# HKUST-KnowComp/DualMessagePassing

Hardware: AMD Instinct MI355X
Metric: (pattern,graph) pairs/sec DMPNN fwd+bwd hid=128 (higher is better)
Workload: dtype f32

## Files before the change

### dualmessagepassing_amd/_abi.py

```python
import ctypes

c_int = ctypes.c_int
c_i32 = ctypes.c_int32
c_i64 = ctypes.c_int64
c_u64 = ctypes.c_uint64
c_f32 = ctypes.c_float
c_double = ctypes.c_double
c_ptr = ctypes.c_void_p
c_size = ctypes.c_size_t

ABI_VERSION = 91

DMP_COLLATE_MAX_JOBS = 4
DMP_POOL_MAX_JOBS = 4
DMP_REDUCE_MAX_SEGMENTS = 16
DMP_ADAMW_MAX_SKIP = 16
DMP_ADAMW_MAX_SEGMENTS = 1024
DMP_LOOKUP_MAX_JOBS = 8
DMP_CONCAT_MAX_JOBS = 12
DMP_GEMM_MAX_JOBS = 12
DMP_GEMM_MAX_TERMS = 3
DMP_ATB_MAX_JOBS = 8
DMP_MEM_MEAN, DMP_MEM_SUM, DMP_MEM_MAX = 0, 1, 2


class dmp_collate_job(ctypes.Structure):
# ... 80 lines not shown

class dmp_head_io(ctypes.Structure):
    _fields_ = [("ps", c_ptr), ("ld_ps", c_i64), ("gs", c_ptr), ("ld_gs", c_i64), ("pl", c_ptr), ("gl", c_ptr), ("scale_p", c_f32),
                ("scale_g", c_f32), ("F", c_ptr), ("Y1S", c_ptr), ("y", c_ptr)]


class dmp_head_grads(ctypes.Structure):
    _fields_ = [("dy", c_ptr), ("dy_scale", c_ptr), ("dY1", c_ptr), ("dP", c_ptr), ("dG", c_ptr), ("dps", c_ptr), ("ld_dps", c_i64),
                ("dgs", c_ptr), ("ld_dgs", c_i64), ("dWp", c_ptr), ("dbp", c_ptr), ("dWg", c_ptr), ("dbg", c_ptr), ("dW1", c_ptr),
                ("db1", c_ptr), ("dW2", c_ptr), ("db2", c_ptr)]


class dmp_typed_job(ctypes.Structure):
    _fields_ = [("Hin", c_ptr), ("ldh", c_i64), ("W2", c_ptr), ("ldw", c_i64), ("w_in_out", c_int), ("bias", c_ptr), ("R", c_ptr),
                ("ldr", c_i64), ("R2", c_ptr), ("ldr2", c_i64), ("act", c_int), ("slope", c_f32), ("out", c_ptr), ("ldo", c_i64)]


class dmp_atb2_job(ctypes.Structure):
    _fields_ = [("Z", c_ptr), ("ldz", c_i64), ("D", c_ptr), ("ldd", c_i64), ("partial_T", c_ptr), ("partial_B", c_ptr),
                ("partial_stride", c_i64), ("ldp", c_int)]


class dmp_atb_job(ctypes.Structure):
    _fields_ = [("A", c_ptr), ("lda", c_i64), ("B", c_ptr), ("ldb", c_i64), ("gate", c_ptr), ("partial", c_ptr), ("partial_stride", c_i64),
                ("ldp", c_int), ("partial_colsum", c_ptr), ("cs_ld", c_int), ("rowmask", c_ptr)]


_p = ctypes.POINTER


# ... 159 lines not shown
    "dmp_l0_bwd_w_rows": (c_int, [c_ptr, c_i64, c_int, c_ptr, c_ptr, c_i64, c_ptr, c_i64, c_ptr, c_ptr, c_i64, c_int, c_ptr, c_ptr]),
    "dmp_typed_partial_rows": (c_i64, [c_i64, c_int]),
    "dmp_out_fwd_typed": (c_int, [_p(dmp_typed_job), c_int, c_ptr, c_ptr, c_ptr, c_i64, c_i64, c_int, c_ptr]),
    "dmp_bwd_h1_typed": (c_int, [c_ptr, c_i64, c_ptr, c_i64, c_ptr, c_i64, c_ptr, c_ptr, c_ptr, c_i64, c_i64, c_int, c_f32, c_ptr, c_i64,
                                 c_ptr, c_ptr, c_ptr]),
    "dmp_kept_rows_jobs": (c_int, [_p(dmp_kept_job), c_int, c_ptr, c_ptr, c_ptr, c_ptr, c_i64, c_ptr, c_ptr, c_ptr, c_ptr]),
    "dmp_row_mask_bits_jobs": (c_int, [_p(dmp_rowmask_job), c_int, c_ptr]),
    "dmp_atb2_blocks": (c_i64, [c_i64, c_int]),
    "dmp_atb2_jobs": (c_int, [_p(dmp_atb2_job), c_int, c_ptr, c_ptr, c_ptr, c_i64, c_i64, c_int, c_ptr]),
    "dmp_bwd_z_w": (c_int, [c_ptr, c_i64, c_ptr, c_i64, c_ptr, c_i64, c_ptr, c_i64, c_i64, c_ptr, c_i64, c_ptr, c_ptr, c_f32, c_f32,
                            c_ptr, c_ptr, c_ptr, c_i64, c_i64, c_int, c_ptr, c_i64, c_ptr, c_i64, c_ptr, c_ptr]),
    "dmp_out_fwd_typed_codes": (c_int, [_p(dmp_typed_job), c_ptr, c_i64, c_int, c_ptr, c_i64, c_i64, c_i64, c_ptr, c_ptr, c_ptr, c_i64, c_i64, c_int, c_ptr]),
    "dmp_bwd_h1_w_blocks": (c_i64, [c_i64]),
    "dmp_bwd_h1_w": (c_int, [c_ptr, c_i64, c_ptr, c_i64, c_ptr, c_i64, c_ptr, c_ptr, c_i64, c_i64, c_int, c_f32, c_ptr, c_i64,
                             c_ptr, c_ptr, c_ptr, c_ptr]),
    "dmp_row_mask_bits": (c_int, [c_ptr, c_i64, c_ptr, c_ptr]),
    "dmp_row_mask_rows": (c_int, [c_ptr, c_i64, c_int, c_i64, c_ptr, c_ptr]),
    "dmp_bwd_z_fused": (c_int, [c_ptr, c_i64, c_ptr, c_i64, c_ptr, c_i64, c_i64, c_ptr, c_i64, c_ptr, c_ptr, c_ptr,
                                c_f32, c_f32, c_i64, c_int, c_ptr, c_i64, c_ptr]),
    "dmp_gemm_k128": (c_int, [c_ptr, c_i64, c_ptr, c_i64, c_int, c_ptr, c_i64, c_i64, c_int, c_ptr]),
    "dmp_edge_combine": (c_int, [c_ptr, c_i64, c_ptr, c_i64, c_ptr, c_ptr, c_ptr, c_ptr, c_ptr, c_i64,
                                 c_int, c_int, c_f32, c_ptr, c_i64, c_ptr]),
    "dmp_relu_bwd_g_colsum": (c_int, [c_ptr, c_i64, c_ptr, c_i64, c_ptr, c_ptr, c_i64, c_int, c_f32, c_ptr, c_i64,
                                      c_ptr, c_ptr]),
    "dmp_edge_combine_bwd_g": (c_int, [c_ptr, c_i64, c_ptr, c_ptr, c_i64, c_int, c_ptr, c_i64, c_ptr]),
    "dmp_compgcn_agg": (c_int, [c_ptr, c_i64, c_ptr, c_i64, c_ptr, c_ptr, c_ptr, c_ptr, c_i64, c_int, c_int,
                                c_ptr, c_i64, c_ptr]),
    "dmp_compgcn_agg_bwd": (c_int, [c_ptr, c_i64, c_ptr, c_i64, c_ptr, c_i64, c_ptr, c_ptr, c_ptr, c_ptr,
                                    c_i64, c_int, c_int, c_ptr, c_i64, c_ptr, c_i64, c_ptr]),
    "dmp_attn_supported_dh": (c_int, [c_int]),
# ... 24 lines not shown
```

### dualmessagepassing_amd/_build.py

```python
import fcntl
import hashlib
import os
import shutil
import subprocess
import tempfile

_HERE = os.path.dirname(os.path.abspath(__file__))
CSRC = os.path.join(_HERE, "csrc")
LIB_PATH = os.path.join(CSRC, "libdmp_hip.so")
HASH_PATH = LIB_PATH + ".srchash"
SOURCES = ["dmp_agg.hip", "dmp_segacc.hip", "dmp_compact.hip", "dmp_graph.hip", "dmp_fused.hip", "dmp_mfma.hip", "dmp_typed.hip", "dmp_h1w.hip", "dmp_atb.hip", "dmp_fold.hip", "dmp_heads.hip", "dmp_layer0.hip", "dmp_bn.hip", "dmp_attn.hip", "dmp_mem.hip", "dmp_cnn.hip", "dmp_rnn.hip", "dmp_relconv.hip", "dmp_relcorr.hip",
           "dmp_subiso.cpp"]
HEADERS = ["dmp_common.h", "dmp_mfma_common.h", os.path.join("..", "..", "include", "dmp_hip.h")]
ARCH = "gfx950"
FLAGS = ["-O3", "-std=c++17", "-fPIC", "-ffp-contract=off", "-Wall", "-Wno-unused-function"]


def find_hipcc():
    for cand in (os.environ.get("HIPCC"), shutil.which("hipcc"), "/opt/rocm/bin/hipcc"):
        if cand and os.path.exists(cand):
            return cand
    return None


def source_hash():
    h = hashlib.sha256()
# ... 61 lines not shown
```

### dualmessagepassing_amd/fused.py

```python
import threading

import torch
from torch.autograd.function import once_differentiable

from . import _abi, _lib, ops
from ._lib import check, ptr, stream_ptr


def _partials(rows, H, dev):
    lib = _lib.load()
    return torch.empty((int(lib.dmp_colsum_partial_rows(rows, H)), H), dtype=torch.float32, device=dev)


MAX_REDUCE_SEGMENTS = _abi.DMP_REDUCE_MAX_SEGMENTS


class _Deferred(threading.local):

    def __init__(self):
        self.stack = []


_deferred = _Deferred()

# ... 657 lines not shown

def bwd_h1_typed(d_o, W2, h1, tiles, slope=0.0, out=None):
    lib = _lib.load()
    E, H = d_o.shape
    slot_edge, tile_scale, num_tiles, bound = tiles
    d_g = out if out is not None else dead_rows_buffer((E, H), d_o.device)
    G = int(lib.dmp_typed_partial_rows(bound, H))
    part = torch.empty((G, H), dtype=torch.float32, device=d_o.device)
    part_rows = torch.empty_like(part)
    W2 = W2.contiguous()
    with _lib.timed("bwd_h1_typed[H=%d,E=%d]", (H, E), 12 * H * E + 4 * E):
        check(lib.dmp_bwd_h1_typed(ptr(d_o), d_o.stride(0), ptr(W2), W2.size(1), ptr(h1), h1.stride(0), ptr(slot_edge), ptr(tile_scale),
                                   ptr(num_tiles), bound, E, H, slope, ptr(d_g), d_g.stride(0), ptr(part), ptr(part_rows), stream_ptr()),
              "dmp_bwd_h1_typed")
    return d_g, reduce_partials(part), reduce_partials(part_rows)


def h1w_ok(d_o, h1, H):
    lib = _lib.load()
    return (H == 128 and not lib.dmp_dev_get_exact_fp32() and d_o.size(0) * d_o.stride(0) * 4 < (1 << 32) - 65536
            and h1.size(0) * h1.stride(0) * 4 < (1 << 32) - 65536 and d_o.size(0) * H * 4 < (1 << 32) - 65536)


def bwd_h1_w(d_o, W2, h1, tiles, slope=0.0, out=None):
    lib = _lib.load()
    E, H = d_o.shape
    slot_edge, _, num_tiles, bound = tiles
    d_g = out if out is not None else dead_rows_buffer((E, H), d_o.device)
    G = int(lib.dmp_bwd_h1_w_blocks(bound))
    part = torch.empty((G, H), dtype=torch.float32, device=d_o.device)
# ... 704 lines not shown
    @staticmethod
    def forward(ctx, index, coef, residual, x, z, v_gate, e_gate, Bn, bn, Wx, Wes, be, nW2, nb2, eW2, eb2,
                WesT=None, nW2t=None, eW2t=None, slope=0.0, vpool=None, epool=None, l0=None, W0=None, WV0=None, edge_rows=True,
                inner=0):
        _lib.require_gpu(x, z)
        H = Bn.size(1)
        x, z = x.contiguous(), z.contiguous()
        Bn, Wx, Wes = Bn.contiguous(), Wx.contiguous(), Wes.contiguous()
        N = index.num_nodes
        from . import side
        side.wait("nodes")
        nd = node_rows(index, v_gate, H) if (N >= 4096 and onepanel_ok(H)) else None
        if nd is not None and l0 is not None and any(n0 % 32 for _, _, (n0, _) in l0.tables(z.size(0), N)):
            nd = None
        S0 = M0 = tables = None
        if l0 is not None:
            enc0, K0 = l0.enc, l0.K
            tables = l0.tables(z.size(0), N)
            if nd is not None and enc0.size(1) % 4 == 0:
                S0 = ops.seg_sum_raw(enc0, index.in_ptr, index.in_ent, N, None, True, -1.0, 1.0,
                                     out=dead_rows_buffer((N, 2 * enc0.size(1)), z.device), rows=nd.rows, tag="seg_sum2_codes")
            else:
                S0 = ops.seg_sum_raw(enc0, index.in_ptr, index.in_ent, N, None, True, -1.0, 1.0)
            Kp = enc0.size(1)
            vcodes_f = l0.venc is not None
            node_pass = (vcodes_f and H in MFMA_WIDTHS and l0.VK + 2 * K0 <= L0_NODE_MAX_COLS and W0.size(0) // K0 <= 2)
            TK = W0.size(0)
            M0 = torch.empty((TK, 2 * H), dtype=torch.float32, device=z.device)
            jobs = [(M0, [(W0, False, Wes, False)], None)]
            if node_pass:
# ... 28 lines not shown
                        SB[n0:n1].addmm_(S0[n0:n1, Kp:Kp + K0], WB[1, t * K0:(t + 1) * K0])
            S = None
        else:
            side.wait("keepcsr")
            kc = keep_in_csr(index, e_gate) if zero_rows_gate(e_gate) else None
            if kc is not None and nd is not None:
                S = ops.seg_sum_raw(z, kc[0], kc[1], N, None, True, -1.0, 1.0, out=dead_rows_buffer((N, 2 * H), z.device), rows=nd.rows)
            elif kc is not None:
                S = ops.seg_sum_raw(z, kc[0], kc[1], N, None, True, -1.0, 1.0)
            else:
                S = ops.seg_sum_raw(z, index.in_ptr, index.in_ent, N, e_gate.reshape(-1) if zero_rows_gate(e_gate) else None, True, -1.0, 1.0)
            if nd is None:
                SB = S @ Bn
        if l0 is None and nd is not None:
            T = nd.tiles
            XP = dead_rows_buffer((N, 3 * H), z.device)
            T1 = dead_rows_buffer((N, H), z.device)
            H1n = dead_rows_buffer((N, H), z.device)
            typed_jobs([dict(a=x, W=Wx[:, :H], bias=bn, out=XP[:, :H]), dict(a=S[:, :H], W=Bn[:H], out=T1),
                        dict(a=x, W=Wx[:, H:2 * H], out=XP[:, H:2 * H]), dict(a=x, W=Wx[:, 2 * H:], out=XP[:, 2 * H:])], T)
            out_fwd_typed(S[:, H:], Bn[H:], None, XP[:, :H], T, out=H1n, slope=slope, prev2=T1)
        elif l0 is not None and node_pass:
            pass
        elif l0 is not None and l0.venc is not None:
            VK = l0.VK
            XP = torch.empty((N, 3 * H), dtype=torch.float32, device=z.device)
            for t, (n0, n1) in l0.vtables(N):
                smallk_embed(l0.venc[n0:n1, :VK], MV[t * VK:(t + 1) * VK], None, XP[n0:n1], H)
        else:
            XP = x @ Wx
        if l0 is not None and node_pass:
            PXr, ldpx = PX, 2 * H
        else:
            PXr, ldpx = XP[:, H:], 3 * H
            if l0 is not None or nd is None:
                H1n = add_bias_relu_(SB, XP[:, :H], bn, slope)
        if nd is not None:
            xn = dead_rows_buffer((N, H), z.device) if (inner & 1) else torch.zeros((N, H), dtype=torch.float32, device=z.device)
            if nW2t is not None:
                out_fwd_typed(H1n, nW2t, nb2, x if residual else None, nd.tiles, out=xn)
            else:
                out_fwd_typed(H1n, nW2, nb2, x if residual else None, nd.tiles, out=xn, w_in_out=False)
        elif onepanel_ok(H):
            xn = out_fwd_mfma(H1n, nW2, nb2, v_gate, x if residual else None, nW2t)
        else:
            xn = gate_residual(x if residual else None, torch.addmm(nb2, H1n, nW2.t()), v_gate)
        sums_only = epool is not None and not edge_rows
        zn = None
        side.wait("erows" if l0 is not None else "tiles")
        dead_gate = e_gate if (SKIP_DEAD_ROWS and USE_ROW_MASKS and e_gate is not None and typed_ok(index, H)
                               and gate_row_mask(e_gate) is not None) else None
        if l0 is not None:
# ... 22 lines not shown
                if l0 is not None and residual and getattr(l0, "z_from_codes", False) and out_codes_ok(H1e, l0.enc, l0.K, W0[-l0.K:]):
                    zn = out_fwd_typed_codes(H1e, eW2t, eb2, l0.enc, l0.K, W0[-l0.K:], tl_, prev=l0.z_head, row0=l0.z_head.size(0))
                else:
                    zn = out_fwd_typed(H1e, eW2t, eb2, l0_rows(l0, W0, z) if residual else None, tl_)
            elif (l0 is not None and residual and e_gate is None and getattr(l0, "z_from_codes", False) and eW2t is not None
                  and out_codes_ok(H1e, l0.enc, l0.K, W0[-l0.K:]) and identity_tiles(H1e.size(0), H1e.device) is not None):
                zn = out_fwd_typed_codes(H1e, eW2t, eb2, l0.enc, l0.K, W0[-l0.K:], identity_tiles(H1e.size(0), H1e.device), prev=l0.z_head,
                                         row0=l0.z_head.size(0))
            else:
                zn = out_fwd_mfma(H1e, eW2, eb2, e_gate, l0_rows(l0, W0, z) if residual else None, eW2t, dead_rows=dead)
        ctx.index, ctx.coef, ctx.residual, ctx.H = index, coef, residual, H
        ctx.v_gate, ctx.e_gate, ctx.WesT, ctx.slope = v_gate, e_gate, WesT, slope
        ctx.vpool, ctx.epool = vpool, epool
        ctx.inner = int(inner)
        ctx.nd = nd
        ctx.l0, ctx.l0_S0, ctx.l0_tables = l0, S0, tables
        ctx.l0_W = None if l0 is None else (W0.detach(), None if WV0 is None else WV0.detach())
        ctx.save_for_backward(x, z if l0 is None else None, S, H1n, H1e, Bn, Wx, Wes, nW2, eW2)
        if vpool is None and epool is None:
            return xn, zn
        ctx.set_materialize_grads(False)
        vs = pool_rows(xn, vpool) if vpool is not None else None
        if sums_only:
            halves = 2 if epool.flag8 is not None else 1
            G_ = epool.num_graphs
            Q = pool_rows(H1e, epool, e_gate).view(G_ * halves, H)
            cnt = pool_weight_sums(epool, e_gate)
            ctx.gcnt = cnt
            cnt = cnt.view(G_ * halves, 1)
            zs = pool_rows(z, epool, e_gate if zero_rows_gate(e_gate) else None).view(G_ * halves, H) if residual else None
# ... 102 lines not shown
                XX = (torch.empty if full else torch.zeros)((TK, (3 if ctx.residual else 2) * H), dtype=torch.float32, device=dG.device)
                for t, rows, _ in tables:
                    if rows[1] > rows[0]:
                        l0_bwd_w(l0.enc, K0, ix.edge_select(coef)[2], dG, dzn if ctx.residual else None, rows, XX[t * K0:(t + 1) * K0],
                                 mask=(gate_row_mask(ctx.e_gate) if (getattr(l0, "enc_mask", None) is not None and binary_gate_mask(ctx.e_gate) is not None)
                                       else getattr(l0, "enc_mask", None)))
                dWes = None
            else:
                fuse_dzw = bool(typed and ctx.needs_input_grad[4] and H == 128 and
                                (ctx.e_gate is None or (SKIP_DEAD_ROWS and zero_rows_gate(ctx.e_gate) and live_tiles(ix, coef, ctx.e_gate) is not None)))
                dWes = None if fuse_dzw else (atb_typed(z, dG, coef, ix, gate=ctx.e_gate) if typed else atb(z, dG))
            wg = (lambda a, b: atb_rows(a, b, colsum=False)[0]) if atb_ok(x, dXP) else atb
            one_launch = onepanel_ok(H) and atb_ok(dxn, H1n) and atb_ok(x, dXP) and (l0 is not None or atb_ok(S, dXP))
            if nd is not None and not (one_launch and binary_gate_mask(ctx.v_gate) is not None):
                raise _lib.DmpError("fused layer backward: the kept-node path needs the masked weight-gradient launch")
            if nd is not None:
                dPn, dbn, db2n = bwd_h1_typed(dxn, nW2, H1n, nd.tiles, slope, out=dXP[:, :H])
                if vcodes:
                    dW2n = atb_rows(dxn, H1n, ctx.v_gate, colsum=False)[0]
            elif onepanel_ok(H) and atb_ok(dxn, H1n):
                if binary_gate_mask(ctx.v_gate) is not None:
                    dPn, dbn, db2n = bwd_h1_mfma(dxn, nW2, H1n, both_halves=False, gate=ctx.v_gate, out=dXP[:, :H], slope=slope,
                                                 rows_colsum=True)
                    if not one_launch or vcodes:
                        dW2n = atb_rows(dxn, H1n, ctx.v_gate, colsum=False)[0]
                else:
                    if not one_launch or vcodes:
                        dW2n, db2n = atb_rows(dxn, H1n, ctx.v_gate)
                    dPn, dbn = bwd_h1_mfma(dxn, nW2, H1n, both_halves=False, gate=ctx.v_gate, out=dXP[:, :H], slope=slope)
            else:
                dOn, db2n = scale_rows_colsum(dxn, ctx.v_gate)
# ... 26 lines not shown
                        klist = nd.rows if (nd is not None and n0 == 0 and n1 == N) else None
                        smallk_atb_cols(l0.venc[n0:n1, :VK], dXP[n0:n1], dxn[n0:n1] if ctx.residual else None,
                                        Yn[:, t * VK:(t + 1) * VK], H,
                                        mask=vmask[n0 // 32:] if (klist is None and vmask is not None and n0 % 32 == 0) else None, rows=klist)
                elif one_launch:
                    vm = binary_gate_mask(ctx.v_gate)
                    if nd is not None:
                        (dW2n, _), (dWx, _) = atb_rows_multi([(dxn, H1n, None, False), (x, dXP, None, False)], tiles=nd.tiles)
                    elif vm is not None:
                        (dW2n, _), (dWx, _) = atb_rows_multi([(dxn, H1n, None, False, vm), (x, dXP, None, False)])
                    else:
                        (dW2n, db2n), (dWx, _) = atb_rows_multi([(dxn, H1n, ctx.v_gate, True, gate_row_mask(ctx.v_gate)), (x, dXP, None, False)])
                else:
                    dWx = wg(x, dXP)
            else:
                if nd is not None:
                    dS = dead_rows_buffer((N, 2 * H), x.device)
                    jobs = [dict(a=dPn, W=Bn[:H], w_in_out=False, out=dS[:, :H]), dict(a=dPn, W=Bn[H:], w_in_out=False, out=dS[:, H:])]
                    if ctx.needs_input_grad[3]:
                        dxU = dead_rows_buffer((N, 2 * H), x.device)
                        jobs += [dict(a=dXP[:, :H], W=Wx[:, :H], w_in_out=False, prev=dxn if ctx.residual else None, out=dxU[:, :H]),
                                 dict(a=dXP[:, H:2 * H], W=Wx[:, H:2 * H], w_in_out=False, out=dxU[:, H:])]
                    typed_jobs(jobs, nd.tiles)
                else:
                    dS = dPn @ Bn.t()
                if one_launch:
                    vm = gate_row_mask(ctx.v_gate)
                    if nd is not None:
                        (dW2n, _), (dBn, _), (dWx, _) = atb_rows_multi([(dxn, H1n, None, False), (S, dPn, None, False), (x, dXP, None, False)],
                                                                        tiles=nd.tiles)
                    elif binary_gate_mask(ctx.v_gate) is not None:
                        (dW2n, _), (dBn, _), (dWx, _) = atb_rows_multi([(dxn, H1n, None, False, vm), (S, dPn, None, False, vm),
                                                                         (x, dXP, None, False)])
                    else:
                        (dW2n, db2n), (dBn, _), (dWx, _) = atb_rows_multi([(dxn, H1n, ctx.v_gate, True, vm), (S, dPn, None, False, vm),
                                                                            (x, dXP, None, False)])
                else:
                    dBn = wg(S, dPn)
                    dWx = wg(x, dXP)
            dx = None
            if ctx.needs_input_grad[3] and nd is not None:
                dx = dead_rows_buffer((N, H), x.device) if (ctx.inner & 2) else torch.zeros((N, H), dtype=torch.float32, device=x.device)
                if l0 is None:
                    out_fwd_typed(dXP[:, 2 * H:], Wx[:, 2 * H:], None, dxU[:, :H], nd.tiles, out=dx, w_in_out=False, prev2=dxU[:, H:])
                else:
                    for b3 in range(3):
                        out_fwd_typed(dXP[:, b3 * H:(b3 + 1) * H], Wx[:, b3 * H:(b3 + 1) * H], None,
                                      (dxn if ctx.residual else None) if b3 == 0 else dx, nd.tiles, out=dx, w_in_out=False)
            elif ctx.needs_input_grad[3]:
                dx = torch.addmm(dxn, dXP, Wx.t()) if ctx.residual else dXP @ Wx.t()
            dz = None
            if l0 is None and ctx.needs_input_grad[4]:
                dead_dz = (("leave" if (ctx.inner & 2) else "zero") if (typed and SKIP_DEAD_ROWS and zero_rows_gate(ctx.e_gate)) else None)
                dst_m = None if nd is None else nd.sel[2]
                both = None
                if typed and dWes is None:
# ... 88 lines not shown
```

### include/dmp_hip.h

```cpp
#ifndef DMP_HIP_H
#define DMP_HIP_H

#include <stddef.h>
#include <stdint.h>

#ifdef __cplusplus
extern "C" {
#endif

#define DMP_OK 0
#define DMP_ERR_BAD_ARG (-1)
#define DMP_ERR_UNSUPPORTED (-2)
#define DMP_ERR_HIP (-3)

#define DMP_ABI_VERSION 91
int dmp_abi_version(void);
const char *dmp_last_hip_error(void);


size_t dmp_csr_workspace_words(int64_t num_nodes, int64_t num_edges);

int dmp_csr_build(const int64_t *key, const uint8_t *flag, int64_t num_edges,
                  int64_t num_nodes, int32_t *rowptr, int32_t *ent,
                  int32_t *key32, int64_t *degree, int32_t *status,
                  int32_t *ws, void *stream);

size_t dmp_csr_pair_workspace_words(int64_t num_nodes);
int dmp_csr_build_pair(const int64_t *dst, const int64_t *src, const uint8_t *flag, int64_t num_edges, int64_t num_nodes,
                       int32_t *in_ptr, int32_t *in_ent, int32_t *dst32, int64_t *in_deg,
                       int32_t *out_ptr, int32_t *out_ent, int32_t *src32, int64_t *out_deg,
// ... 469 lines not shown
  float *partial_T, *partial_B; int64_t partial_stride; int ldp;
} dmp_atb2_job;
int64_t dmp_atb2_blocks(int64_t tiles_bound, int num_jobs);
int dmp_atb2_jobs(const dmp_atb2_job *jobs, int num_jobs, const int32_t *slot_row, const float *tile_scale, const int32_t *num_tiles,
                  int64_t tiles_bound, int64_t rows, int H, void *stream);

int dmp_bwd_z_w(const float *dPre, int64_t ldp, const float *Z, int64_t ldz, const float *W, int64_t ldw, const float *D, int64_t ldd,
                int64_t num_nodes, const float *base, int64_t ldb, const int32_t *dst, const uint8_t *flag, float s0, float s1,
                const int32_t *slot_edge, const float *tile_scale, const int32_t *num_tiles, int64_t tiles_bound, int64_t E, int H,
                const int32_t *base_map, int64_t base_rows, float *dZ, int64_t ldo, float *partial_w, void *stream);
int64_t dmp_bwd_h1_w_blocks(int64_t tiles_bound);
int dmp_bwd_h1_w(const float *dO, int64_t ldo, const float *W2, int64_t ldw, const float *H1, int64_t ldh,
                 const int32_t *slot_edge, const int32_t *num_tiles, int64_t tiles_bound, int64_t E, int H, float slope,
                 float *dG, int64_t ldg, float *partial, float *partial_rows, float *partial_w, void *stream);

int dmp_bwd_z_fused(const float *dPre, int64_t ldp, const float *W, int64_t ldw,
                    const float *D, int64_t ldd, int64_t num_nodes, const float *base, int64_t ldb,
                    const float *coefE, const int32_t *dst, const uint8_t *flag, float s0,
                    float s1, int64_t num_edges, int H, float *dZ, int64_t ldz, void *stream);

int dmp_edge_fwd_typed(const float *Z, int64_t ldz, const float *W, int64_t ldw, const float *P,
                       int64_t ldp, int64_t num_nodes, const float *bias, const int32_t *selA,
                       const int32_t *selB, const int32_t *slot_edge, const float *tile_scale,
                       const int32_t *num_tiles, int64_t tiles_bound, int64_t num_edges, int H,
                       float slope, float *H1, int64_t ldh, void *stream);
int dmp_mask_slots(const int32_t *slot, int64_t n, const float *gate, int64_t E, int32_t *out, void *stream);
int dmp_bwd_z_typed_arow(const float *dPre, int64_t ldp, const float *W, int64_t ldw, const float *D, int64_t ldd,
                         int64_t num_nodes, const float *base, int64_t ldb, const int32_t *dst, const uint8_t *flag,
                         float s0, float s1, const int32_t *slot_edge, const int32_t *slot_arow, const float *tile_scale,
                         const int32_t *num_tiles, int64_t tiles_bound, int64_t E, int H, int w_transposed,
// ... 93 lines not shown
```

Measured before the change: 469,800.

## Fuse node-side typed GEMM chain into single persistent MFMA kernel for fwd and bwd

Adds a node_chain kernel that runs the whole per-node chain (x/S projections, bias+activation, second linear layer with residual) for each 128-row tile in one launch. It keeps intermediates in LDS as split-bf16 images and streams packed weight panels double-buffered. In backward it also fuses activation-gradient, dS/dx products and column sums. This replaces several typed_jobs/out_fwd_typed launches and their intermediate global round-trips, at the cost of a large LDS footprint, limited occupancy, and an extra weight-packing pass each call.

After: 486,500, median of 6. +3.5%, better.

```diff
diff --git a/dualmessagepassing_amd/_abi.py b/dualmessagepassing_amd/_abi.py
--- a/dualmessagepassing_amd/_abi.py
+++ b/dualmessagepassing_amd/_abi.py
@@ -9,7 +9,7 @@
 c_ptr = ctypes.c_void_p
 c_size = ctypes.c_size_t
 
-ABI_VERSION = 91
+ABI_VERSION = 92
 
 DMP_COLLATE_MAX_JOBS = 4
 DMP_POOL_MAX_JOBS = 4
@@ -120,6 +120,10 @@
 class dmp_typed_job(ctypes.Structure):
     _fields_ = [("Hin", c_ptr), ("ldh", c_i64), ("W2", c_ptr), ("ldw", c_i64), ("w_in_out", c_int), ("bias", c_ptr), ("R", c_ptr),
                 ("ldr", c_i64), ("R2", c_ptr), ("ldr2", c_i64), ("act", c_int), ("slope", c_f32), ("out", c_ptr), ("ldo", c_i64)]
+
+
+class dmp_chain_panel(ctypes.Structure):
+    _fields_ = [("W", c_ptr), ("ld", c_i64), ("transposed", c_int)]
 
 
 class dmp_atb2_job(ctypes.Structure):
@@ -309,6 +313,13 @@
     "dmp_bwd_h1_w_blocks": (c_i64, [c_i64]),
     "dmp_bwd_h1_w": (c_int, [c_ptr, c_i64, c_ptr, c_i64, c_ptr, c_i64, c_ptr, c_ptr, c_i64, c_i64, c_int, c_f32, c_ptr, c_i64,
                              c_ptr, c_ptr, c_ptr, c_ptr]),
+    "dmp_node_chain_blocks": (c_i64, [c_i64]),
+    "dmp_node_chain_panel_words": (c_i64, []),
+    "dmp_node_chain_pack": (c_int, [_p(dmp_chain_panel), c_int, c_ptr, c_ptr]),
+    "dmp_node_chain_fwd": (c_int, [c_ptr, c_i64, c_ptr, c_i64, c_ptr, c_ptr, c_ptr, c_int, c_f32, c_ptr, c_ptr, c_i64, c_i64, c_int,
+                                   c_ptr, c_i64, c_ptr, c_i64, c_ptr, c_i64, c_ptr]),
+    "dmp_node_chain_bwd": (c_int, [c_ptr, c_i64, c_ptr, c_i64, c_ptr, c_i64, c_ptr, c_int, c_f32, c_ptr, c_ptr, c_i64, c_i64, c_int,
+                                   c_ptr, c_i64, c_ptr, c_i64, c_ptr, c_i64, c_ptr, c_ptr, c_ptr]),
     "dmp_row_mask_bits": (c_int, [c_ptr, c_i64, c_ptr, c_ptr]),
     "dmp_row_mask_rows": (c_int, [c_ptr, c_i64, c_int, c_i64, c_ptr, c_ptr]),
     "dmp_bwd_z_fused": (c_int, [c_ptr, c_i64, c_ptr, c_i64, c_ptr, c_i64, c_i64, c_ptr, c_i64, c_ptr, c_ptr, c_ptr,
diff --git a/dualmessagepassing_amd/_build.py b/dualmessagepassing_amd/_build.py
--- a/dualmessagepassing_amd/_build.py
+++ b/dualmessagepassing_amd/_build.py
@@ -9,7 +9,7 @@
 CSRC = os.path.join(_HERE, "csrc")
 LIB_PATH = os.path.join(CSRC, "libdmp_hip.so")
 HASH_PATH = LIB_PATH + ".srchash"
-SOURCES = ["dmp_agg.hip", "dmp_segacc.hip", "dmp_compact.hip", "dmp_graph.hip", "dmp_fused.hip", "dmp_mfma.hip", "dmp_typed.hip", "dmp_h1w.hip", "dmp_atb.hip", "dmp_fold.hip", "dmp_heads.hip", "dmp_layer0.hip", "dmp_bn.hip", "dmp_attn.hip", "dmp_mem.hip", "dmp_cnn.hip", "dmp_rnn.hip", "dmp_relconv.hip", "dmp_relcorr.hip",
+SOURCES = ["dmp_agg.hip", "dmp_segacc.hip", "dmp_compact.hip", "dmp_graph.hip", "dmp_fused.hip", "dmp_mfma.hip", "dmp_typed.hip", "dmp_h1w.hip", "dmp_nodechain.hip", "dmp_atb.hip", "dmp_fold.hip", "dmp_heads.hip", "dmp_layer0.hip", "dmp_bn.hip", "dmp_attn.hip", "dmp_mem.hip", "dmp_cnn.hip", "dmp_rnn.hip", "dmp_relconv.hip", "dmp_relcorr.hip",
            "dmp_subiso.cpp"]
 HEADERS = ["dmp_common.h", "dmp_mfma_common.h", os.path.join("..", "..", "include", "dmp_hip.h")]
 ARCH = "gfx950"
diff --git a/dualmessagepassing_amd/csrc/dmp_nodechain.hip b/dualmessagepassing_amd/csrc/dmp_nodechain.hip
--- /dev/null
+++ b/dualmessagepassing_amd/csrc/dmp_nodechain.hip
@@ -0,0 +1,418 @@
+#include "dmp_mfma_common.h"
+
+namespace dmp {
+__device__ int llvm_struct_buffer_load_i32(i32x4 rsrc, int vindex, int voffset, int soffset, int aux) __asm("llvm.amdgcn.struct.buffer.load.i32");
+__device__ void llvm_struct_buffer_store_i32(int data, i32x4 rsrc, int vindex, int voffset, int soffset, int aux) __asm("llvm.amdgcn.struct.buffer.store.i32");
+namespace {
+
+constexpr int kChainThreads = 512;
+constexpr int kChainRows = 128;
+constexpr int kChainStrideD = 68;
+constexpr int kChainPlane = kChainRows * kChainStrideD;
+constexpr int kChainImageBytes = 3 * kChainPlane * 4;
+constexpr int kChainPanelBytes = 3 * 128 * 128 * 2;
+constexpr int kChainChunkBytes = kChainPanelBytes / 4;
+constexpr int kChainLdsBytes = kChainImageBytes + 2 * kChainChunkBytes + kChainRows * 4;
+constexpr int kChainMaxPanels = 12;
+
+__device__ __forceinline__ float sbuf_load1(srsrc_t r, int row, uint32_t col_bytes) {
+  return __int_as_float(llvm_struct_buffer_load_i32(r, row, (int)col_bytes, 0, 0));
+}
+__device__ __forceinline__ void sbuf_store1(float v, srsrc_t r, int row, uint32_t col_bytes) {
+  llvm_struct_buffer_store_i32(__float_as_int(v), r, row, (int)col_bytes, 0, 0);
+}
+
+struct PackArgs {
+  const float *W[kChainMaxPanels];
+  int64_t ld[kChainMaxPanels];
+  int transposed[kChainMaxPanels];
+  uint32_t *out;
+};
+__global__ __launch_bounds__(256) void chain_pack_k(PackArgs p) {
+  const int item = (int)blockIdx.x * 256 + (int)threadIdx.x;
+  const int lane = item & 63, cb = (item >> 6) & 3, g = item >> 8;
+  const int li = lane & 31, h = lane >> 5;
+  const float *W = nullptr;
+  int64_t ld = 0;
+  int tr = 0;
+#pragma unroll
+  for (int j = 0; j < kChainMaxPanels; ++j)
+    if (j == (int)blockIdx.y) { W = p.W[j]; ld = p.ld[j]; tr = p.transposed[j]; }
+  const int k0 = 64 * h + 8 * g, c = 32 * cb + li;
+  float w[8];
+#pragma unroll
+  for (int j = 0; j < 8; ++j) w[j] = tr ? W[(int64_t)c * ld + k0 + j] : W[(int64_t)(k0 + j) * ld + c];
+  Split8 s;
+  split8(make_float4(w[0], w[1], w[2], w[3]), make_float4(w[4], w[5], w[6], w[7]), s);
+  uint32_t *o = p.out + (size_t)blockIdx.y * (kChainPanelBytes / 4) + (size_t)g * 3072 + cb * 256 + lane * 4;
+  *reinterpret_cast<uint4 *>(o) = make_uint4(s.hi.u[0], s.hi.u[1], s.hi.u[2], s.hi.u[3]);
+  *reinterpret_cast<uint4 *>(o + 1024) = make_uint4(s.mid.u[0], s.mid.u[1], s.mid.u[2], s.mid.u[3]);
+  *reinterpret_cast<uint4 *>(o + 2048) = make_uint4(s.lo.u[0], s.lo.u[1], s.lo.u[2], s.lo.u[3]);
+}
+
+struct ChainArgs {
+  const float *A0, *A1, *A2;
+  int64_t lda0, lda1, lda2;
+  const float *X; int64_t ldx;
+  const float *Res; int64_t ldres;
+  const float *bias1, *bias2;
+  float *O0, *O1, *O2, *O3;
+  int64_t ldo0, ldo1, ldo2, ldo3;
+  float *partial, *partialA;
+  const uint32_t *panels;
+  int npanels;
+  const int32_t *slot; const int32_t *num_tiles;
+  int64_t rows;
+  float slope;
+};
+
+template <bool BWD, bool FULL>
+__global__ __launch_bounds__(kChainThreads) void node_chain_k(ChainArgs p) {
+  extern __shared__ __attribute__((aligned(256))) unsigned char lds[];
+  uint32_t *Aimg = reinterpret_cast<uint32_t *>(lds);
+  unsigned char *Pb = lds + kChainImageBytes;
+  int *ids_s = reinterpret_cast<int *>(lds + kChainImageBytes + 2 * kChainChunkBytes);
+
+  const int t = threadIdx.x;
+  const int wave = __builtin_amdgcn_readfirstlane(t >> 6);
+  const int lane = t & 63, li = lane & 31, h = lane >> 5;
+  const int rt = wave >> 1, ch = wave & 1;
+  const int q = t & 31, r0 = t >> 5;
+  const float slope = __builtin_bit_cast(float, __builtin_amdgcn_readfirstlane(__builtin_bit_cast(int, p.slope)));
+  const bool has_res = p.Res != nullptr;
+  const int NC = __builtin_amdgcn_readfirstlane(p.npanels) * 4;
+  constexpr bool full = FULL;
+
+  const int ntiles = __builtin_amdgcn_readfirstlane(*p.num_tiles);
+  const int chunk = (ntiles + (int)gridDim.x - 1) / (int)gridDim.x;
+  const int lo = (int)blockIdx.x * chunk;
+  const int hi = lo + chunk < ntiles ? lo + chunk : ntiles;
+  if (hi <= lo) {
+    if (BWD && t < 128) { p.partial[(int64_t)blockIdx.x * 128 + t] = 0.f; p.partialA[(int64_t)blockIdx.x * 128 + t] = 0.f; }
+    return;
+  }
+  const rsrc_t rs_slot = make_rsrc(p.slot, (uint32_t)hi * (kSub * 4u));
+  const rsrc_t rs_pan = make_rsrc(p.panels, (uint32_t)NC * (uint32_t)kChainChunkBytes);
+  const srsrc_t rs_A0 = make_srsrc(p.A0, p.lda0, p.rows), rs_A1 = make_srsrc(p.A1, p.lda1, p.rows), rs_A2 = make_srsrc(p.A2, p.lda2, p.rows);
+  const srsrc_t rs_X = make_srsrc(p.X, p.X ? p.ldx : (int64_t)128, p.X ? p.rows : 0);
+  const srsrc_t rs_Res = make_srsrc(p.Res, has_res ? p.ldres : (int64_t)128, has_res ? p.rows : 0);
+  const srsrc_t rs_O0 = make_srsrc(p.O0, p.ldo0, p.rows), rs_O1 = make_srsrc(p.O1, p.ldo1, p.rows), rs_O2 = make_srsrc(p.O2, p.ldo2, p.rows);
+  const srsrc_t rs_O3 = make_srsrc(p.O3, p.O3 ? p.ldo3 : (int64_t)128, p.O3 ? p.rows : 0);
+
+  int ids[8];
+  float4 pre[8];
+  auto load_ids = [&](int tile0) {
+#pragma unroll
+    for (int m = 0; m < 8; ++m) {
+      const int idx = tile0 * kSub + r0 + 16 * m;
+      const int v = (int)__builtin_amdgcn_raw_buffer_load_b32(rs_slot, idx * 4, 0, 0);
+      ids[m] = idx < hi * kSub ? v : -1;
+    }
+  };
+  auto load_rows = [&](srsrc_t rs) {
+#pragma unroll
+    for (int m = 0; m < 8; ++m) pre[m] = sbuf_load4(rs, ids[m], (uint32_t)q * 16u);
+  };
+  float4 csA = make_float4(0.f, 0.f, 0.f, 0.f);
+  auto stage = [&](bool first) {
+#pragma unroll
+    for (int m = 0; m < 8; ++m) {
+      const int row = r0 + 16 * m;
+      if (BWD && first) { csA.x += pre[m].x; csA.y += pre[m].y; csA.z += pre[m].z; csA.w += pre[m].w; }
+      uint2 ph, pm, pl;
+      split_pair(pre[m].x, pre[m].y, ph.x, pm.x, pl.x);
+      split_pair(pre[m].z, pre[m].w, ph.y, pm.y, pl.y);
+      uint32_t *d = Aimg + row * kChainStrideD + q * 2;
+      *reinterpret_cast<uint2 *>(d) = ph;
+      *reinterpret_cast<uint2 *>(d + kChainPlane) = pm;
+      *reinterpret_cast<uint2 *>(d + 2 * kChainPlane) = pl;
+      if (first && q == 0) ids_s[row] = ids[m];
+    }
+  };
+
+  f32x16 acc[2];
+  auto zero_acc = [&]() {
+#pragma unroll
+    for (int r = 0; r < 16; ++r) { acc[0][r] = 0.f; acc[1][r] = 0.f; }
+  };
+  auto product = [&](int pidx) {
+#pragma unroll
+    for (int cc = 0; cc < 4; ++cc) {
+      const int c = 4 * pidx + cc;
+      const int nc = c + 1 == NC ? 0 : c + 1;
+      uint4 pc[3];
+#pragma unroll
+      for (int i = 0; i < 3; ++i) {
+        const u32x4 v = __builtin_amdgcn_raw_buffer_load_b128(rs_pan, (i * kChainThreads + t) * 16, nc * kChainChunkBytes, 0);
+        pc[i] = make_uint4(v.x, v.y, v.z, v.w);
+      }
+      const unsigned char *pb = Pb + (cc & 1) * kChainChunkBytes;
+      const uint32_t *ar = Aimg + (32 * rt + li) * kChainStrideD + 32 * h;
+#pragma unroll
+      for (int gl = 0; gl < 2; ++gl) {
+        const int g = 2 * cc + gl;
+        Split8 a;
+        a.hi.v = *reinterpret_cast<const bf16x8 *>(ar + 4 * g);
+        a.mid.v = *reinterpret_cast<const bf16x8 *>(ar + kChainPlane + 4 * g);
+        a.lo.v = *reinterpret_cast<const bf16x8 *>(ar + 2 * kChainPlane + 4 * g);
+#pragma unroll
+        for (int cbl = 0; cbl < 2; ++cbl) {
+          const unsigned char *bq = pb + gl * 12288 + (2 * ch + cbl) * 1024 + lane * 16;
+          Split8 b;
+          b.hi.v = *reinterpret_cast<const bf16x8 *>(bq);
+          b.mid.v = *reinterpret_cast<const bf16x8 *>(bq + 4096);
+          b.lo.v = *reinterpret_cast<const bf16x8 *>(bq + 8192);
+          acc[cbl] = mfma_x6(a, b, acc[cbl]);
+        }
+      }
+      uint4 *pw = reinterpret_cast<uint4 *>(Pb + ((cc + 1) & 1) * kChainChunkBytes);
+#pragma unroll
+      for (int i = 0; i < 3; ++i) pw[i * kChainThreads + t] = pc[i];
+      lds_barrier();
+    }
+  };
+  int rid[16];
+  auto store_acc = [&](srsrc_t rs) {
+#pragma unroll
+    for (int cb = 0; cb < 2; ++cb)
+#pragma unroll
+      for (int r = 0; r < 16; ++r) sbuf_store1(acc[cb][r], rs, rid[r], (uint32_t)(64 * ch + 32 * cb + li) * 4u);
+  };
+  auto acc_to_image = [&]() {
+#pragma unroll
+    for (int cb = 0; cb < 2; ++cb)
+#pragma unroll
+      for (int i = 0; i < 8; ++i) {
+        const float va = acc[cb][2 * i], vb = acc[cb][2 * i + 1];
+        const float got = __shfl_xor((li & 1) ? va : vb, 1, 64);
+        const float f0 = (li & 1) ? got : va, f1 = (li & 1) ? vb : got;
+        const int r = 2 * i + (li & 1);
+        const int row = 32 * rt + (r & 3) + 8 * (r >> 2) + 4 * h;
+        uint32_t ph, pm, pl;
+        split_pair(f0, f1, ph, pm, pl);
+        uint32_t *d = Aimg + row * kChainStrideD + 32 * ch + 16 * cb + (li >> 1);
+        d[0] = ph; d[kChainPlane] = pm; d[2 * kChainPlane] = pl;
+      }
+  };
+  float colsum[2] = {0.f, 0.f};
+
+  load_ids(lo);
+  load_rows(rs_A0);
+  {
+    uint4 *pw = reinterpret_cast<uint4 *>(Pb);
+#pragma unroll
+    for (int i = 0; i < 3; ++i) {
+      const u32x4 v = __builtin_amdgcn_raw_buffer_load_b128(rs_pan, (i * kChainThreads + t) * 16, 0, 0);
+      pw[i * kChainThreads + t] = make_uint4(v.x, v.y, v.z, v.w);
+    }
+  }
+  for (int g0 = lo; g0 < hi; g0 += 4) {
+    stage(true);
+    lds_barrier();
+#pragma unroll
+    for (int qd = 0; qd < 4; ++qd) {
+      const int4 v = *reinterpret_cast<const int4 *>(&ids_s[32 * rt + 8 * qd + 4 * h]);
+      rid[4 * qd] = v.x; rid[4 * qd + 1] = v.y; rid[4 * qd + 2] = v.z; rid[4 * qd + 3] = v.w;
+    }
+    if (!BWD) {
+      load_rows(rs_A1);
+      zero_acc(); product(0); store_acc(rs_O0);
+      zero_acc(); product(1); store_acc(rs_O1);
+      zero_acc(); product(2);
+      stage(false); lds_barrier();
+      load_rows(rs_A2);
+      product(3);
+      stage(false); lds_barrier();
+      load_ids(g0 + 4);
+      product(4);
+      load_rows(rs_A0);
+#pragma unroll
+      for (int cb = 0; cb < 2; ++cb) {
+        const float b = p.bias1[64 * ch + 32 * cb + li];
+#pragma unroll
+        for (int r = 0; r < 16; ++r) acc[cb][r] = act_fwd(acc[cb][r] + b, slope);
+      }
+      float res[2][16];
+#pragma unroll
+      for (int cb = 0; cb < 2; ++cb)
+#pragma unroll
+        for (int r = 0; r < 16; ++r) res[cb][r] = sbuf_load1(rs_Res, rid[r], (uint32_t)(64 * ch + 32 * cb + li) * 4u);
+      store_acc(rs_O2);
+      acc_to_image();
+      lds_barrier();
+      zero_acc(); product(5);
+#pragma unroll
+      for (int cb = 0; cb < 2; ++cb) {
+        const float b = p.bias2[64 * ch + 32 * cb + li];
+#pragma unroll
+        for (int r = 0; r < 16; ++r) acc[cb][r] = res[cb][r] + (acc[cb][r] + b);
+      }
+      store_acc(rs_O3);
+    } else {
+      float hv[2][16];
+#pragma unroll
+      for (int cb = 0; cb < 2; ++cb)
+#pragma unroll
+        for (int r = 0; r < 16; ++r) hv[cb][r] = sbuf_load1(rs_X, rid[r], (uint32_t)(64 * ch + 32 * cb + li) * 4u);
+      zero_acc(); product(0);
+      if (full) load_rows(rs_A1);
+      else load_ids(g0 + 4);
+#pragma unroll
+      for (int cb = 0; cb < 2; ++cb)
+#pragma unroll
+        for (int r = 0; r < 16; ++r) {
+          acc[cb][r] = act_bwd(hv[cb][r], acc[cb][r], slope);
+          colsum[cb] += acc[cb][r];
+        }
+      store_acc(rs_O0);
+      acc_to_image();
+      lds_barrier();
+      zero_acc(); product(1);
+      if (!full) load_rows(rs_A0);
+      store_acc(rs_O1);
+      zero_acc(); product(2); store_acc(rs_O2);
+      if (full) {
+        zero_acc(); product(3);
+        stage(false); lds_barrier();
+        load_rows(rs_A2);
+        product(4);
+        stage(false); lds_barrier();
+        load_ids(g0 + 4);
+        float res[2][16];
+#pragma unroll
+        for (int cb = 0; cb < 2; ++cb)
+#pragma unroll
+          for (int r = 0; r < 16; ++r) res[cb][r] = sbuf_load1(rs_Res, rid[r], (uint32_t)(64 * ch + 32 * cb + li) * 4u);
+        product(5);
+        load_rows(rs_A0);
+#pragma unroll
+        for (int cb = 0; cb < 2; ++cb)
+#pragma unroll
+          for (int r = 0; r < 16; ++r) acc[cb][r] = res[cb][r] + acc[cb][r];
+        store_acc(rs_O3);
+      }
+    }
+  }
+  if (BWD) {
+    float *red = reinterpret_cast<float *>(Pb);
+    float *redA = red + 4 * 128;
+#pragma unroll
+    for (int cb = 0; cb < 2; ++cb) {
+      const float s = colsum[cb] + __shfl_xor(colsum[cb], 32, 64);
+      if (h == 0) red[rt * 128 + 64 * ch + 32 * cb + li] = s;
+    }
+    *reinterpret_cast<float4 *>(&redA[r0 * 128 + q * 4]) = csA;
+    lds_barrier();
+    if (t < 128) {
+      float s = red[t];
+#pragma unroll
+      for (int w = 1; w < 4; ++w) s += red[w * 128 + t];
+      p.partial[(int64_t)blockIdx.x * 128 + t] = s;
+      float sa = redA[t];
+#pragma unroll
+      for (int w = 1; w < 16; ++w) sa += redA[w * 128 + t];
+      p.partialA[(int64_t)blockIdx.x * 128 + t] = sa;
+    }
+  }
+}
+
+inline unsigned chain_blocks(int64_t tiles_bound) {
+  const int64_t want = (tiles_bound + 3) / 4;
+  return (unsigned)(want < 1 ? 1 : (want > 256 ? 256 : want));
+}
+
+constexpr int kMaxDevicesC = 64;
+template <bool BWD, bool FULL>
+inline bool chain_lds_ready() {
+  static bool done[kMaxDevicesC] = {};
+  int dev = 0;
+  if (hipGetDevice(&dev) != hipSuccess || dev < 0 || dev >= kMaxDevicesC) dev = 0;
+  if (done[dev]) return true;
+  const hipError_t e = hipFuncSetAttribute(reinterpret_cast<const void *>(&node_chain_k<BWD, FULL>), hipFuncAttributeMaxDynamicSharedMemorySize, kChainLdsBytes);
+  if (e != hipSuccess) { set_last_hip_error(e); return false; }
+  done[dev] = true;
+  return true;
+}
+
+inline bool chain_rows_ok(const float *a, int64_t ld, int64_t rows) {
+  return a && ld >= 128 && ld % 4 == 0 && aligned16(a) && stride_ok(ld) && fits4g(rows, ld);
+}
+
+}
+}
+
+using namespace dmp;
+
+extern "C" {
+
+int64_t dmp_node_chain_blocks(int64_t tiles_bound) { return (int64_t)chain_blocks(tiles_bound); }
+int64_t dmp_node_chain_panel_words(void) { return kChainPanelBytes / 4; }
+
+int dmp_node_chain_pack(const dmp_chain_panel *panels, int num_panels, uint32_t *out, void *stream) {
+  if (!panels || !out || num_panels < 1 || num_panels > kChainMaxPanels || !aligned16(out)) return DMP_ERR_BAD_ARG;
+  PackArgs a{};
+  for (int j = 0; j < num_panels; ++j) {
+    if (!panels[j].W || panels[j].ld < 128) return DMP_ERR_BAD_ARG;
+    a.W[j] = panels[j].W; a.ld[j] = panels[j].ld; a.transposed[j] = panels[j].transposed ? 1 : 0;
+  }
+  a.out = out;
+  chain_pack_k<<<dim3(8, (unsigned)num_panels), 256, 0, (hipStream_t)stream>>>(a);
+  return check_launch();
+}
+
+int dmp_node_chain_fwd(const float *x, int64_t ldx, const float *S, int64_t lds, const uint32_t *panels, const float *bn, const float *b2,
+                       int residual, float slope, const int32_t *slot, const int32_t *num_tiles, int64_t tiles_bound, int64_t rows, int H,
+                       float *H1n, int64_t ldh, float *P, int64_t ldp, float *xn, int64_t ldxn, void *stream) {
+  if (H != 128 || g_exact_fp32) return DMP_ERR_UNSUPPORTED;
+  if (rows < 0 || tiles_bound < 0) return DMP_ERR_BAD_ARG;
+  if (!slope_ok(slope)) return DMP_ERR_UNSUPPORTED;
+  if (rows == 0 || tiles_bound == 0) return DMP_OK;
+  if (!panels || !bn || !b2 || !slot || !num_tiles || !aligned16(panels)) return DMP_ERR_BAD_ARG;
+  if (!x || !S || !H1n || !P || !xn || ldx < H || lds < 2 * H || ldh < H || ldp < 2 * H || ldxn < H) return DMP_ERR_BAD_ARG;
+  if (!chain_rows_ok(x, ldx, rows) || !chain_rows_ok(S, lds, rows) || !chain_rows_ok(H1n, ldh, rows) || !chain_rows_ok(P, ldp, rows) ||
+      !chain_rows_ok(xn, ldxn, rows) || rows >= ((int64_t)1 << 30) || tiles_bound * kSub * 4 >= ((int64_t)1 << 32) - 8192)
+    return DMP_ERR_UNSUPPORTED;
+  if (!chain_lds_ready<false, true>()) return DMP_ERR_HIP;
+  ChainArgs a{};
+  a.A0 = x; a.lda0 = ldx; a.A1 = S; a.lda1 = lds; a.A2 = S + H; a.lda2 = lds;
+  a.Res = residual ? x : nullptr; a.ldres = ldx; a.bias1 = bn; a.bias2 = b2;
+  a.O0 = P; a.ldo0 = ldp; a.O1 = P + H; a.ldo1 = ldp; a.O2 = H1n; a.ldo2 = ldh; a.O3 = xn; a.ldo3 = ldxn;
+  a.panels = panels; a.npanels = 6; a.slot = slot; a.num_tiles = num_tiles; a.rows = rows; a.slope = slope;
+  node_chain_k<false, true><<<chain_blocks(tiles_bound), kChainThreads, kChainLdsBytes, (hipStream_t)stream>>>(a);
+  return check_launch();
+}
+
+int dmp_node_chain_bwd(const float *dxn, int64_t ldd, const float *H1n, int64_t ldh, const float *dP, int64_t ldp, const uint32_t *panels,
+                       int residual, float slope, const int32_t *slot, const int32_t *num_tiles, int64_t tiles_bound, int64_t rows, int H,
+                       float *dPn, int64_t ldn, float *dS, int64_t lds, float *dx, int64_t ldx, float *partial, float *partial_rows,
+                       void *stream) {
+  if (H != 128 || g_exact_fp32) return DMP_ERR_UNSUPPORTED;
+  if (rows < 0 || tiles_bound < 0) return DMP_ERR_BAD_ARG;
+  if (!slope_ok(slope)) return DMP_ERR_UNSUPPORTED;
+  if (!partial || !partial_rows) return DMP_ERR_BAD_ARG;
+  hipStream_t st = (hipStream_t)stream;
+  if (rows == 0 || tiles_bound == 0) {
+    const size_t bytes = sizeof(float) * 128 * (size_t)chain_blocks(tiles_bound);
+    if (hipMemsetAsync(partial, 0, bytes, st) != hipSuccess || hipMemsetAsync(partial_rows, 0, bytes, st) != hipSuccess) return DMP_ERR_HIP;
+    return DMP_OK;
+  }
+  if (!panels || !slot || !num_tiles || !aligned16(panels)) return DMP_ERR_BAD_ARG;
+  if (!dxn || !H1n || !dPn || !dS || ldd < H || ldh < H || ldn < H || lds < 2 * H || (dx && (!dP || ldp < 2 * H || ldx < H))) return DMP_ERR_BAD_ARG;
+  if (!chain_rows_ok(dxn, ldd, rows) || !chain_rows_ok(H1n, ldh, rows) || !chain_rows_ok(dPn, ldn, rows) || !chain_rows_ok(dS, lds, rows) ||
+      (dx && (!chain_rows_ok(dP, ldp, rows) || !chain_rows_ok(dx, ldx, rows))) || rows >= ((int64_t)1 << 30) ||
+      tiles_bound * kSub * 4 >= ((int64_t)1 << 32) - 8192)
+    return DMP_ERR_UNSUPPORTED;
+  if (!(dx ? chain_lds_ready<true, true>() : chain_lds_ready<true, false>())) return DMP_ERR_HIP;
+  ChainArgs a{};
+  a.A0 = dxn; a.lda0 = ldd;
+  a.A1 = dx ? dP : dxn; a.lda1 = dx ? ldp : ldd; a.A2 = dx ? dP + H : dxn; a.lda2 = a.lda1;
+  a.X = H1n; a.ldx = ldh; a.Res = (dx && residual) ? dxn : nullptr; a.ldres = ldd;
+  a.O0 = dPn; a.ldo0 = ldn; a.O1 = dS; a.ldo1 = lds; a.O2 = dS + H; a.ldo2 = lds; a.O3 = dx; a.ldo3 = ldx;
+  a.partial = partial; a.partialA = partial_rows;
+  a.panels = panels; a.npanels = dx ? 6 : 3; a.slot = slot; a.num_tiles = num_tiles; a.rows = rows; a.slope = slope;
+  if (dx) node_chain_k<true, true><<<chain_blocks(tiles_bound), kChainThreads, kChainLdsBytes, st>>>(a);
+  else node_chain_k<true, false><<<chain_blocks(tiles_bound), kChainThreads, kChainLdsBytes, st>>>(a);
+  return check_launch();
+}
+
+}
diff --git a/dualmessagepassing_amd/fused.py b/dualmessagepassing_amd/fused.py
--- a/dualmessagepassing_amd/fused.py
+++ b/dualmessagepassing_amd/fused.py
@@ -695,6 +695,71 @@
                                    ptr(num_tiles), bound, E, H, slope, ptr(d_g), d_g.stride(0), ptr(part), ptr(part_rows), stream_ptr()),
               "dmp_bwd_h1_typed")
     return d_g, reduce_partials(part), reduce_partials(part_rows)
+
+
+USE_NODE_CHAIN = True
+
+
+def node_chain_ok(H, *tensors):
+    if not USE_NODE_CHAIN or H != 128 or _lib.load().dmp_dev_get_exact_fp32():
+        return False
+    lim = (1 << 32) - 65536
+    for a in tensors:
+        if a is None:
+            continue
+        if (a.dtype != torch.float32 or a.dim() != 2 or a.stride(1) != 1 or a.stride(0) % 4 or a.stride(0) * 4 > 16383
+                or a.data_ptr() % 16 or a.size(0) * a.stride(0) * 4 >= lim):
+            return False
+    return True
+
+
+def node_chain_panels(Bn, Wx, nW2):
+    lib = _lib.load()
+    H = Bn.size(1)
+    Bn, Wx, nW2 = Bn.detach(), Wx.detach(), nW2.detach()
+    _lib.require_gpu(Bn, Wx, nW2)
+    if not (Bn.is_contiguous() and Wx.is_contiguous() and nW2.is_contiguous()):
+        raise _lib.DmpError("node_chain_panels: contiguous weights expected")
+    words = int(lib.dmp_node_chain_panel_words())
+    out = torch.empty(12 * words, dtype=torch.int32, device=Bn.device)
+    e = Bn.element_size()
+    spec = [(Wx.data_ptr() + H * e, 3 * H, 0), (Wx.data_ptr() + 2 * H * e, 3 * H, 0), (Wx.data_ptr(), 3 * H, 0),
+            (Bn.data_ptr(), H, 0), (Bn.data_ptr() + H * H * e, H, 0), (nW2.data_ptr(), H, 1),
+            (nW2.data_ptr(), H, 0), (Bn.data_ptr(), H, 1), (Bn.data_ptr() + H * H * e, H, 1),
+            (Wx.data_ptr(), 3 * H, 1), (Wx.data_ptr() + H * e, 3 * H, 1), (Wx.data_ptr() + 2 * H * e, 3 * H, 1)]
+    J = (_abi.dmp_chain_panel * len(spec))()
+    for j, (w, ld, tr) in zip(J, spec):
+        j.W, j.ld, j.transposed = w, ld, tr
+    check(lib.dmp_node_chain_pack(J, len(spec), ptr(out), stream_ptr()), "dmp_node_chain_pack")
+    return out[:6 * words], out[6 * words:]
+
+
+def node_chain_fwd(x, S, panels, bn, b2, residual, slope, tiles, H1n, P, xn):
+    lib = _lib.load()
+    slot, _, num_tiles, bound = tiles
+    R, H = x.shape
+    _lib.require_gpu(x, S, panels, bn, b2, H1n, P, xn)
+    with _lib.timed("out_fwd_typed[H=%d,R=%d,jobs=2]", (H, R), 4 * H * R * 6):
+        check(lib.dmp_node_chain_fwd(ptr(x), x.stride(0), ptr(S), S.stride(0), ptr(panels), ptr(bn), ptr(b2), int(bool(residual)), float(slope),
+                                     ptr(slot), ptr(num_tiles), bound, R, H, ptr(H1n), H1n.stride(0), ptr(P), P.stride(0), ptr(xn), xn.stride(0),
+                                     stream_ptr()), "dmp_node_chain_fwd")
+    return H1n, P, xn
+
+
+def node_chain_bwd(dxn, H1n, dP, panels, residual, slope, tiles, dPn, dS, dx=None):
+    lib = _lib.load()
+    slot, _, num_tiles, bound = tiles
+    R, H = dxn.shape
+    _lib.require_gpu(dxn, H1n, dP, panels, dPn, dS, dx)
+    G = int(lib.dmp_node_chain_blocks(bound))
+    part = torch.empty((G, H), dtype=torch.float32, device=dxn.device)
+    part_rows = torch.empty_like(part)
+    with _lib.timed("out_fwd_typed[H=%d,R=%d,jobs=2]", (H, R), 4 * H * R * 6):
+        check(lib.dmp_node_chain_bwd(ptr(dxn), dxn.stride(0), ptr(H1n), H1n.stride(0), ptr(dP), dP.stride(0) if dP is not None else 2 * H,
+                                     ptr(panels), int(bool(residual)), float(slope), ptr(slot), ptr(num_tiles), bound, R, H,
+                                     ptr(dPn), dPn.stride(0), ptr(dS), dS.stride(0), ptr(dx), dx.stride(0) if dx is not None else H,
+                                     ptr(part), ptr(part_rows), stream_ptr()), "dmp_node_chain_bwd")
+    return reduce_partials(part), reduce_partials(part_rows)
 
 
 def h1w_ok(d_o, h1, H):
@@ -1429,6 +1494,7 @@
         if nd is not None and l0 is not None and any(n0 % 32 for _, _, (n0, _) in l0.tables(z.size(0), N)):
             nd = None
         S0 = M0 = tables = None
+        chained, chain_panels = False, None
         if l0 is not None:
             enc0, K0 = l0.enc, l0.K
             tables = l0.tables(z.size(0), N)
@@ -1487,12 +1553,19 @@
                 SB = S @ Bn
         if l0 is None and nd is not None:
             T = nd.tiles
-            XP = dead_rows_buffer((N, 3 * H), z.device)
-            T1 = dead_rows_buffer((N, H), z.device)
             H1n = dead_rows_buffer((N, H), z.device)
-            typed_jobs([dict(a=x, W=Wx[:, :H], bias=bn, out=XP[:, :H]), dict(a=S[:, :H], W=Bn[:H], out=T1),
-                        dict(a=x, W=Wx[:, H:2 * H], out=XP[:, H:2 * H]), dict(a=x, W=Wx[:, 2 * H:], out=XP[:, 2 * H:])], T)
-            out_fwd_typed(S[:, H:], Bn[H:], None, XP[:, :H], T, out=H1n, slope=slope, prev2=T1)
+            chained = node_chain_ok(H, x, S, Bn, Wx, nW2)
+            if chained:
+                PX = dead_rows_buffer((N, 2 * H), z.device)
+                xn = dead_rows_buffer((N, H), z.device) if (inner & 1) else torch.zeros((N, H), dtype=torch.float32, device=z.device)
+                chain_panels = node_chain_panels(Bn, Wx, nW2)
+                node_chain_fwd(x, S, chain_panels[0], bn, nb2, residual, slope, T, H1n, PX, xn)
+            else:
+                XP = dead_rows_buffer((N, 3 * H), z.device)
+                T1 = dead_rows_buffer((N, H), z.device)
+                typed_jobs([dict(a=x, W=Wx[:, :H], bias=bn, out=XP[:, :H]), dict(a=S[:, :H], W=Bn[:H], out=T1),
+                            dict(a=x, W=Wx[:, H:2 * H], out=XP[:, H:2 * H]), dict(a=x, W=Wx[:, 2 * H:], out=XP[:, 2 * H:])], T)
+                out_fwd_typed(S[:, H:], Bn[H:], None, XP[:, :H], T, out=H1n, slope=slope, prev2=T1)
         elif l0 is not None and node_pass:
             pass
         elif l0 is not None and l0.venc is not None:
@@ -1502,13 +1575,15 @@
                 smallk_embed(l0.venc[n0:n1, :VK], MV[t * VK:(t + 1) * VK], None, XP[n0:n1], H)
         else:
             XP = x @ Wx
-        if l0 is not None and node_pass:
+        if (l0 is not None and node_pass) or chained:
             PXr, ldpx = PX, 2 * H
         else:
             PXr, ldpx = XP[:, H:], 3 * H
             if l0 is not None or nd is None:
                 H1n = add_bias_relu_(SB, XP[:, :H], bn, slope)
-        if nd is not None:
+        if chained:
+            pass
+        elif nd is not None:
             xn = dead_rows_buffer((N, H), z.device) if (inner & 1) else torch.zeros((N, H), dtype=torch.float32, device=z.device)
             if nW2t is not None:
                 out_fwd_typed(H1n, nW2t, nb2, x if residual else None, nd.tiles, out=xn)
@@ -1561,6 +1636,7 @@
         ctx.vpool, ctx.epool = vpool, epool
         ctx.inner = int(inner)
         ctx.nd = nd
+        ctx.chain_panels = chain_panels
         ctx.l0, ctx.l0_S0, ctx.l0_tables = l0, S0, tables
         ctx.l0_W = None if l0 is None else (W0.detach(), None if WV0 is None else WV0.detach())
         ctx.save_for_backward(x, z if l0 is None else None, S, H1n, H1e, Bn, Wx, Wes, nW2, eW2)
@@ -1693,7 +1769,16 @@
             one_launch = onepanel_ok(H) and atb_ok(dxn, H1n) and atb_ok(x, dXP) and (l0 is not None or atb_ok(S, dXP))
             if nd is not None and not (one_launch and binary_gate_mask(ctx.v_gate) is not None):
                 raise _lib.DmpError("fused layer backward: the kept-node path needs the masked weight-gradient launch")
-            if nd is not None:
+            chained = (nd is not None and l0 is None and ctx.chain_panels is not None
+                       and node_chain_ok(H, dxn, H1n, dXP))
+            dx = None
+            if chained:
+                dPn = dXP[:, :H]
+                dS = dead_rows_buffer((N, 2 * H), x.device)
+                if ctx.needs_input_grad[3]:
+                    dx = dead_rows_buffer((N, H), x.device) if (ctx.inner & 2) else torch.zeros((N, H), dtype=torch.float32, device=x.device)
+                dbn, db2n = node_chain_bwd(dxn, H1n, dXP[:, H:], ctx.chain_panels[1], ctx.residual, slope, nd.tiles, dPn, dS, dx)
+            elif nd is not None:
                 dPn, dbn, db2n = bwd_h1_typed(dxn, nW2, H1n, nd.tiles, slope, out=dXP[:, :H])
                 if vcodes:
                     dW2n = atb_rows(dxn, H1n, ctx.v_gate, colsum=False)[0]
@@ -1750,7 +1835,9 @@
                 else:
                     dWx = wg(x, dXP)
             else:
-                if nd is not None:
+                if chained:
+                    pass
+                elif nd is not None:
                     dS = dead_rows_buffer((N, 2 * H), x.device)
                     jobs = [dict(a=dPn, W=Bn[:H], w_in_out=False, out=dS[:, :H]), dict(a=dPn, W=Bn[H:], w_in_out=False, out=dS[:, H:])]
                     if ctx.needs_input_grad[3]:
@@ -1774,8 +1861,9 @@
                 else:
                     dBn = wg(S, dPn)
                     dWx = wg(x, dXP)
-            dx = None
-            if ctx.needs_input_grad[3] and nd is not None:
+            if chained:
+                pass
+            elif ctx.needs_input_grad[3] and nd is not None:
                 dx = dead_rows_buffer((N, H), x.device) if (ctx.inner & 2) else torch.zeros((N, H), dtype=torch.float32, device=x.device)
                 if l0 is None:
                     out_fwd_typed(dXP[:, 2 * H:], Wx[:, 2 * H:], None, dxU[:, :H], nd.tiles, out=dx, w_in_out=False, prev2=dxU[:, H:])
diff --git a/include/dmp_hip.h b/include/dmp_hip.h
--- a/include/dmp_hip.h
+++ b/include/dmp_hip.h
@@ -13,7 +13,7 @@
 #define DMP_ERR_UNSUPPORTED (-2)
 #define DMP_ERR_HIP (-3)
 
-#define DMP_ABI_VERSION 91
+#define DMP_ABI_VERSION 92
 int dmp_abi_version(void);
 const char *dmp_last_hip_error(void);
 
@@ -513,6 +513,20 @@
                  const int32_t *slot_edge, const int32_t *num_tiles, int64_t tiles_bound, int64_t E, int H, float slope,
                  float *dG, int64_t ldg, float *partial, float *partial_rows, float *partial_w, void *stream);
 
+typedef struct {
+  const float *W; int64_t ld; int transposed;
+} dmp_chain_panel;
+int64_t dmp_node_chain_blocks(int64_t tiles_bound);
+int64_t dmp_node_chain_panel_words(void);
+int dmp_node_chain_pack(const dmp_chain_panel *panels, int num_panels, uint32_t *out, void *stream);
+int dmp_node_chain_fwd(const float *x, int64_t ldx, const float *S, int64_t lds, const uint32_t *panels, const float *bn, const float *b2,
+                       int residual, float slope, const int32_t *slot, const int32_t *num_tiles, int64_t tiles_bound, int64_t rows, int H,
+                       float *H1n, int64_t ldh, float *P, int64_t ldp, float *xn, int64_t ldxn, void *stream);
+int dmp_node_chain_bwd(const float *dxn, int64_t ldd, const float *H1n, int64_t ldh, const float *dP, int64_t ldp, const uint32_t *panels,
+                       int residual, float slope, const int32_t *slot, const int32_t *num_tiles, int64_t tiles_bound, int64_t rows, int H,
+                       float *dPn, int64_t ldn, float *dS, int64_t lds, float *dx, int64_t ldx, float *partial, float *partial_rows,
+                       void *stream);
+
 int dmp_bwd_z_fused(const float *dPre, int64_t ldp, const float *W, int64_t ldw,
                     const float *D, int64_t ldd, int64_t num_nodes, const float *base, int64_t ldb,
                     const float *coefE, const int32_t *dst, const uint8_t *flag, float s0,
```
